# lukecq1231/nats

Hardware: NVIDIA H100
Metric: decoder tokens/sec (dim=1000, src=400, |V|=30k) @1/2/4/8 H100 vs Theano CPU (higher is better)
Workload: dtype f32

## Files before the change

### nats_b200/csrc/api.cu

```cuda
#include <stdarg.h>
#include <stdlib.h>

#include <vector>

#include "model.cuh"

namespace nats {
static thread_local char g_err[1024] = "";
void set_error(const char* fmt, ...) {
    va_list ap;
    va_start(ap, fmt);
    vsnprintf(g_err, sizeof(g_err), fmt, ap);
    va_end(ap);
}
}

namespace nats {
namespace {
struct ProfRec { int cls; double flops, bytes; };
struct ProfState {
    bool on = false;
    std::vector<cudaEvent_t> ev;
    std::vector<ProfRec> recs;
};
// ... 312 lines not shown

int64_t nats_sampler_workspace_bytes(const nats_dims_t* dims, int Tx, int n) {
    if (check_dims(dims) != 0 || Tx < 1 || n < 1) return -1;
    return carve_sampler(*dims, Tx, n, nullptr).bytes;
}

int nats_sampler_init(nats_ctx_t* ctx, void* stream, const nats_dims_t* dims, const float* params, const int64_t* x,
                      const float* x_mask, int Tx, int n, void* ws, int64_t ws_bytes, float* init_state, float* ctx_out,
                      float* pctx_out) {
    NATS_REQUIRE(ctx && ws && params && x && init_state && ctx_out, "null argument");
    NATS_TRY(check_dims(dims));
    NATS_REQUIRE(Tx >= 1 && n >= 1, "shape");
    const SamplerWS w = carve_sampler(*dims, Tx, n, ws);
    NATS_REQUIRE(ws_bytes >= w.bytes, "workspace too small (see nats_sampler_workspace_bytes)");
    cudaStream_t st = reinterpret_cast<cudaStream_t>(stream);
    EncBufs e;
    memset(&e, 0, sizeof(e));
    e.emb_x = w.emb_x;
    e.xproj[0] = w.xproj[0]; e.xproj[1] = w.xproj[1];
    e.cc = ctx_out; e.ctxsum = w.ctxsum; e.xlen = w.xlen; e.xinv = w.xinv; e.ctx_mean = w.ctx_mean;
    e.init_state = init_state; e.part_a = w.part_a;
    e.gemm_scratch = w.gemm_scratch; e.gemm_scratch_floats = w.gemm_scratch_floats;
    e.enc_scratch = w.enc_scratch; e.enc_scratch_floats = w.enc_scratch_floats;
    e.enc_counters = w.enc_counters; e.enc_counter_ints = w.enc_counter_ints;
    NATS_TRY(encoder_forward(ctx, st, *dims, params, x, x_mask, Tx, n, e));
    if (pctx_out) {
        const ParamOff o = param_offsets(*dims);
        const int A = dims->dim_att, C = 2 * dims->dim;
        GemmProblem p = gemm_problem(ctx_out, C, params + o.Wc_att, A, pctx_out, A, Tx * n, A, C);
        p.bias = params + o.b_att;
        NATS_TRY(gemm_auto(ctx, st, p, false, false, w.gemm_scratch, w.gemm_scratch_floats));
    }
    return 0;
}

}

namespace {

int sampler_next(nats_ctx_t* ctx, void* stream, const nats_dims_t* dims, const float* params, const int64_t* y,
                 const float* ctx_in, int64_t ctx_tstride, int64_t ctx_bstride, const float* pctx_in,
                 int64_t pctx_tstride, int64_t pctx_bstride, int rows_per_src, const int32_t* src_len, const float* state,
                 const float* acc_ctx, const float* acc_alpha, int Tx, int n, uint64_t rng_seed, uint64_t rng_step, void* ws,
                 int64_t ws_bytes, float* probs, int64_t* sample, float* state_out, float* alphaT, float* ctxs,
                 float* acc_ctx_out, float* acc_alpha_out) {
    NATS_REQUIRE(ctx && ws && params && y && ctx_in && state && acc_ctx && acc_alpha, "null argument");
    NATS_REQUIRE(probs && state_out && alphaT && ctxs && acc_ctx_out && acc_alpha_out, "null output");
// ... 225 lines not shown
```

### nats_b200/csrc/enc_tc.cu

```cuda
#include <cuda.h>

#include "ops.cuh"
#include "tc_common.cuh"

namespace nats {

namespace {

using namespace tc;

constexpr int kMmaWG = 3;
constexpr int kMmaThreads = kMmaWG * 128;
constexpr int kProdWarp = kMmaWG * 4;
constexpr int kGateWarp0 = kProdWarp + 1;
constexpr int kGateThreads = 256;
constexpr int kThreads = kGateWarp0 * 32 + kGateThreads;
constexpr int kMaxRows = 64 * kMmaWG;
constexpr int kMaxNS = 8;
constexpr int kMaxWords = 12;
constexpr int kMaxDps = 16;
constexpr int kMaxCtasPerDir = 74;
constexpr long long kSpinLimit = 2000000000LL;
constexpr int kCtrStride = 32;

struct EncTc {
    CUtensorMap map_raw[2];
    CUtensorMap map_lo[2];
    const float* Ucat[2];
    const float* mask;
    const float* xproj[2];
    float* cc;
    float* r[2]; float* u[2]; float* c[2]; float* p[2];
    float* ctxsum;
    const float* dcc;
    const float* mean_grad;
    const float* coef;
    float* dG[2]; float* dGx[2];
    float* lo;
    unsigned long long* slab;
    unsigned* bar;
    unsigned long long* dbg;
    int Tx, n, D, Kp;
    int NT, S, dpc, dps, Kc, nkbA, NS, nwg;
};

__device__ __forceinline__ void mbar_wait_b(uint64_t* bar, uint32_t parity) {
    const uint32_t addr = smem_u32(bar);
    const long long t0 = clock64();
    uint32_t ok;
    do {
        asm volatile(
            "{\n\t.reg .pred p;\n\t"
            "mbarrier.try_wait.parity.shared::cta.b64 p, [%1], %2;\n\t"
            "selp.u32 %0, 1, 0, p;\n\t}"
            : "=r"(ok) : "r"(addr), "r"(parity) : "memory");
        if (!ok && clock64() - t0 > kSpinLimit) __trap();
    } while (!ok);
}
__device__ __forceinline__ void flag_arrive(unsigned* ctr) {
    asm volatile("red.release.gpu.global.add.u32 [%0], 1;" ::"l"(ctr) : "memory");
}
// ... 4 lines not shown
__device__ __forceinline__ unsigned long long ld_word(const unsigned long long* p) {
    unsigned long long w;
    asm volatile("ld.relaxed.gpu.global.u64 %0, [%1];" : "=l"(w) : "l"(p) : "memory");
    return w;
}

__device__ __forceinline__ uint32_t a_off(int m, int k, uint32_t kb_bytes) {
    const int kb = k >> 5, kk = k & 31;
    return (uint32_t)kb * kb_bytes + (uint32_t)m * 128u + (uint32_t)(((kk >> 2) ^ (m & 7)) << 4) + (uint32_t)((kk & 3) << 2);
}

template <int BN>
__device__ __forceinline__ void mma_ss(float (&d)[BN / 2], uint64_t da, uint64_t db) {
    if constexpr (BN == 32) wgmma_ss_n32(d, da, db);
    else wgmma_ss_n64(d, da, db);
}
template <int BN>
__device__ __forceinline__ void mma_rs(float (&d)[BN / 2], const uint32_t (&a)[4], uint64_t db) {
    if constexpr (BN == 32) wgmma_rs_n32(d, a, db);
    else wgmma_rs_n64(d, a, db);
}

template <int BN, bool BWD>
__global__ void __launch_bounds__(kThreads, 1) enc_tc_kernel(const __grid_constant__ EncTc a) {
    constexpr uint32_t kStage = 2u * BN * 128u;
    constexpr int EPT = (kMaxDps * BN + kGateThreads - 1) / kGateThreads;
    constexpr int NG = BWD ? 1 : 3;
    constexpr int R = BN / 2;

    extern __shared__ __align__(1024) unsigned char smem[];
    __shared__ __align__(8) uint64_t full[kMaxNS];
    __shared__ __align__(8) uint64_t empty[kMaxNS];

    const int tid = threadIdx.x, warp = __shfl_sync(0xffffffffu, tid >> 5, 0), lane = tid & 31;
    const int D = a.D, n = a.n, Tx = a.Tx, D3 = 3 * a.D, C = 2 * a.D;
    const int S = a.S, NT = a.NT, dpc = a.dpc, dps = a.dps;
    const int dir = blockIdx.x / (NT * S);
    const int rem = blockIdx.x - dir * NT * S;
    const int tile = rem / S, crank = rem - tile * S;
    const int d0 = tile * dpc;
    const int nd = min(dpc, D - d0);
    const int Ktot = BWD ? D3 : D;
    const int kbeg = crank * a.Kc;
    const int kend = min(Ktot, kbeg + a.Kc);
    const int klen = max(0, kend - kbeg);
    const int nkb = (klen + 31) >> 5;
    const int NS = a.NS;
    const uint32_t kb_bytes = (uint32_t)a.nwg * 8192u;

    const uint32_t sA = (smem_u32(smem) + 1023u) & ~1023u;
    const uint32_t sRing = sA + (uint32_t)a.nkbA * kb_bytes;

    {
        const uint32_t words = (uint32_t)a.nkbA * kb_bytes / 4u;
        for (uint32_t i = tid; i < words / 4; i += kThreads)
            asm volatile("st.shared.v4.f32 [%0], {%1,%1,%1,%1};" ::"r"(sA + i * 16u), "f"(0.f) : "memory");
    }
    if (tid == 0) {
        asm volatile("prefetch.tensormap [%0];" ::"l"(&a.map_raw[dir]) : "memory");
        asm volatile("prefetch.tensormap [%0];" ::"l"(&a.map_lo[dir]) : "memory");
        for (int s = 0; s < NS; ++s) { mbar_init(&full[s], 1); mbar_init(&empty[s], kMmaThreads / 32); }
        asm volatile("fence.mbarrier_init.release.cluster;" ::: "memory");
    }
    __syncthreads();
    {
        const float* __restrict__ W = a.Ucat[dir];
        if (!BWD) {
            const int rows = 3 * nd;
            const int total = klen * rows;
            for (int e = tid; e < total; e += kThreads) {
                const int kl = e / rows, mm = e - kl * rows;
                const int g = mm / nd, dl = mm - g * nd;
                const float v = __ldg(W + (long long)(kbeg + kl) * D3 + g * D + d0 + dl);
                asm volatile("st.shared.f32 [%0], %1;" ::"r"(sA + a_off(g * dpc + dl, kl, kb_bytes)), "f"(v) : "memory");
            }
        } else {
            const int total = nd * klen;
            for (int e = tid; e < total; e += kThreads) {
                const int m = e / klen, kl = e - m * klen;
                const float v = __ldg(W + (long long)(d0 + m) * D3 + kbeg + kl);
                asm volatile("st.shared.f32 [%0], %1;" ::"r"(sA + a_off(m, kl, kb_bytes)), "f"(v) : "memory");
            }
        }
    }
    asm volatile("fence.proxy.async.shared::cta;" ::: "memory");
    __syncthreads();

    unsigned* tctr = a.bar + (dir * NT + tile) * kCtrStride;
    const bool stamp = a.dbg != nullptr && blockIdx.x == 0;
#define ENC_STAMP(i) do { a.dbg[i] = gtimer(); a.dbg[32 + (i)] = (unsigned long long)clock64(); } while (0)

    if (warp == kProdWarp) {
        const int kcov = min(Ktot, kbeg + 32 * nkb);
        bool need = false;
        if (lane < NT) {
            const int u0 = lane * dpc, u1 = min(D, u0 + dpc);
            for (int g = 0; g < (BWD ? 3 : 1); ++g) need = need || (g * D + u0 < kcov && g * D + u1 > kbeg);
        }
        const unsigned* pctr = a.bar + (dir * NT + lane) * kCtrStride;
        uint32_t it = 0;
        for (int s = 1; s < Tx; ++s) {
            {
                const unsigned target = (unsigned)(S * (kGateThreads / 32) * s);
                const long long t0 = clock64();
                bool ok;
                do {
                    ok = true;
                    if (need) {
                        unsigned v;
                        asm volatile("ld.acquire.gpu.global.u32 %0, [%1];" : "=r"(v) : "l"(pctr) : "memory");
                        ok = v >= target;
                    }
                    if (!ok && clock64() - t0 > kSpinLimit) __trap();
                } while (!__all_sync(0xffffffffu, ok));
            }
            if (lane == 0) {
                const int brow = BWD ? (dir == 0 ? Tx - s : s - 1) : (dir == 0 ? s - 1 : Tx - s);
                asm volatile("fence.proxy.async;" ::: "memory");
                if (stamp && s == 8) ENC_STAMP(0);
                for (int kb = 0; kb < nkb; ++kb, ++it) {
                    const uint32_t slot = it % (uint32_t)NS;
                    if (it >= (uint32_t)NS) mbar_wait_b(&empty[slot], ((it / (uint32_t)NS) - 1u) & 1u);
                    mbar_expect_tx(&full[slot], kStage);
                    const uint32_t dst = sRing + slot * kStage;
                    tma_load_3d(dst, &a.map_raw[dir], &full[slot], kbeg + 32 * kb, 0, brow);
                    tma_load_3d(dst + BN * 128u, &a.map_lo[dir], &full[slot], kbeg + 32 * kb, 0, (s - 1) & 1);
                }
            }
            __syncwarp();
        }
    } else if (warp < kProdWarp) {
        const int wg = warp >> 2;
        const bool active = wg < a.nwg;
        const int r0 = 64 * wg + 16 * (warp & 3) + (lane >> 2);
        const int q = lane & 3;
        int g_row[2], dl_row[2];
        bool row_ok[2];
        unsigned long long* slab_w[2];
#pragma unroll
        for (int h = 0; h < 2; ++h) {
// ... 43 lines not shown
                    wgmma_commit();
                    wgmma_wait<0>();
                    reg_fence(acc_hh); reg_fence(acc_x);
                }
                __syncwarp();
                if (lane == 0) mbar_arrive(&empty[slot]);
            }
            if (stamp && s == 8 && tid == 0) ENC_STAMP(3);
#pragma unroll
            for (int h = 0; h < 2; ++h) {
                if (!row_ok[h]) continue;
#pragma unroll
                for (int j = 0; j < BN / 8; ++j)
#pragma unroll
                    for (int e = 0; e < 2; ++e) {
                        const int i = 4 * j + 2 * h + e;
                        st_word(slab_w[h] + (long long)(8 * j + 2 * q + e) * dpc, acc_hh[i] + acc_x[i], (uint32_t)s);
                    }
            }
            if (stamp && s == 8 && tid == 0) ENC_STAMP(6);
            asm volatile("bar.arrive 2, %0;" ::"r"(kMmaThreads + kGateThreads) : "memory");
        }
    } else {
        const int gtid = tid - kGateWarp0 * 32;
        const unsigned long long* slab_tile = a.slab + (long long)(dir * NT + tile) * S * NG * BN * dpc;
        const int nw = S * NG;
        const int nds = max(0, min(dps, nd - crank * dps));
        const int dbase = d0 + crank * dps;
        int eb[EPT], ed[EPT];
        bool ev[EPT];
        float carry[EPT], csum[EPT];
#pragma unroll
        for (int i = 0; i < EPT; ++i) {
            const int e = gtid + kGateThreads * i;
            eb[i] = e / dps;
            ed[i] = e - eb[i] * dps;
            ev[i] = eb[i] < n && ed[i] < nds;
            carry[i] = 0.f; csum[i] = 0.f;
        }
        for (int s = 0; s < Tx; ++s) {
            const int pos = BWD ? (dir == 0 ? Tx - 1 - s : s) : (dir == 0 ? s : Tx - 1 - s);
            float x0[EPT], x1[EPT], x2[EPT], mk[EPT];
            float sr_[EPT], su_[EPT], sc_[EPT], sp_[EPT];
#pragma unroll
            for (int i = 0; i < EPT; ++i) {
                x0[i] = x1[i] = x2[i] = 0.f; mk[i] = 1.f;
                sr_[i] = su_[i] = sc_[i] = sp_[i] = 0.f;
                if (ev[i]) {
                    const long long row = (long long)pos * n + eb[i];
                    const int d = dbase + ed[i];
                    if (a.mask) mk[i] = __ldg(a.mask + row);
                    if (!BWD) {
                        const float* xp = a.xproj[dir] + row * D3 + d;
                        x0[i] = __ldg(xp); x1[i] = __ldg(xp + D); x2[i] = __ldg(xp + 2 * D);
                    } else {
                        const long long o = row * D + d;
                        sr_[i] = __ldg(a.r[dir] + o); su_[i] = __ldg(a.u[dir] + o); sc_[i] = __ldg(a.c[dir] + o); sp_[i] = __ldg(a.p[dir] + o);
                        x0[i] = __ldg(a.dcc + row * C + dir * D + d);
                        const int prev = dir == 0 ? pos - 1 : pos + 1;
                        x1[i] = (s < Tx - 1) ? __ldg(a.cc + ((long long)prev * n + eb[i]) * C + dir * D + d) : 0.f;
                        x2[i] = a.mean_grad ? __ldg(a.coef + eb[i]) * __ldg(a.mean_grad + (long long)eb[i] * C + dir * D + d) : 0.f;
                    }
                }
            }
            constexpr bool kDefer = EPT <= 2;
            float o0[kDefer ? EPT : 1], o1[kDefer ? EPT : 1], o2[kDefer ? EPT : 1], o3[kDefer ? EPT : 1];
            auto finish = [&](int i, float s0, float s1, float s2) {
                const long long row = (long long)pos * n + eb[i];
                const int d = dbase + ed[i];
                float q0, q1, q2, q3 = 0.f;
                if (!BWD) {
                    const float r = sigmoidf_(s0 + x0[i]), u = sigmoidf_(s1 + x1[i]);
                    const float cnd = tanhf(s2 * r + x2[i]);
                    const float hn = u * carry[i] + (1.f - u) * cnd;
                    const float h = mk[i] * hn + (1.f - mk[i]) * carry[i];
                    a.cc[row * C + dir * D + d] = h;
                    a.lo[((long long)(dir * 2 + (s & 1)) * n + eb[i]) * a.Kp + d] = resid(h);
                    carry[i] = h;
                    csum[i] += mk[i] * h;
                    q0 = r; q1 = u; q2 = cnd; q3 = s2;
                } else {
                    const float m = mk[i], r = sr_[i], u = su_[i], cnd = sc_[i], pp = sp_[i], hp = x1[i];
                    float dh = x0[i];
                    if (s > 0) { dh += carry[i]; dh += s0; }
                    if (a.mean_grad) dh += m * x2[i];
                    const float dhn = m * dh;
                    const float du = dhn * (hp - cnd);
                    const float dc = dhn * (1.f - u);
                    const float dpc_ = dc * (1.f - cnd * cnd);
                    const float dp = dpc_ * r;
                    const float dr = dpc_ * pp;
                    const float dgr = dr * r * (1.f - r);
                    const float dgu = du * u * (1.f - u);
                    float* g = a.dG[dir] + row * D3 + d;
                    g[0] = dgr; g[D] = dgu; g[2 * D] = dp;
                    float* gl = a.lo + ((long long)(dir * 2 + (s & 1)) * n + eb[i]) * a.Kp + d;
                    gl[0] = resid(dgr); gl[D] = resid(dgu); gl[2 * D] = resid(dp);
                    carry[i] = (1.f - m) * dh + dhn * u;
                    q0 = dgr; q1 = dgu; q2 = dpc_;
                }
// ... 46 lines not shown
                    for (int j = 0; j < 2; ++j) {
                        if (i0 + j < EPT && ev[i0 + j]) {
                            float p0 = 0.f, p1 = 0.f, p2 = 0.f;
#pragma unroll
                            for (int k = 0; k < kMaxWords; k += NG) {
                                if (k < nw) {
                                    p0 += __uint_as_float((uint32_t)w[j][k]);
                                    if (NG == 3) {
                                        p1 += __uint_as_float((uint32_t)w[j][k + NG - 2]);
                                        p2 += __uint_as_float((uint32_t)w[j][k + NG - 1]);
                                    }
                                }
                            }
                            finish(i0 + j, p0, p1, p2);
                        }
                    }
                }
            } else {
#pragma unroll
                for (int i = 0; i < EPT; ++i)
                    if (ev[i]) finish(i, 0.f, 0.f, 0.f);
            }
            if (stamp && s == 8 && gtid == 0) ENC_STAMP(9);
            __syncwarp();
            if (lane == 0) {
                flag_arrive(tctr);
                if (stamp && s == 8 && gtid == 0) ENC_STAMP(5);
            }
            if (kDefer) {
#pragma unroll
                for (int i = 0; i < EPT; ++i) {
                    if (ev[i]) {
                        const long long row = (long long)pos * n + eb[i];
                        const int d = dbase + ed[i];
                        if (!BWD) {
                            if (a.r[dir]) {
                                const long long o = row * D + d;
                                a.r[dir][o] = o0[kDefer ? i : 0]; a.u[dir][o] = o1[kDefer ? i : 0];
                                a.c[dir][o] = o2[kDefer ? i : 0]; a.p[dir][o] = o3[kDefer ? i : 0];
                            }
                        } else {
                            float* gx = a.dGx[dir] + row * D3 + d;
                            gx[0] = o0[kDefer ? i : 0]; gx[D] = o1[kDefer ? i : 0]; gx[2 * D] = o2[kDefer ? i : 0];
                        }
                    }
                }
            }
        }
        if (!BWD && a.ctxsum) {
#pragma unroll
            for (int i = 0; i < EPT; ++i)
                if (ev[i]) a.ctxsum[(long long)eb[i] * C + dir * D + dbase + ed[i]] = csum[i];
        }
    }
}

typedef CUresult (*EncodeTiledFn)(CUtensorMap*, CUtensorMapDataType, cuuint32_t, void*, const cuuint64_t*, const cuuint64_t*,
                                  const cuuint32_t*, const cuuint32_t*, CUtensorMapInterleave, CUtensorMapSwizzle,
                                  CUtensorMapL2promotion, CUtensorMapFloatOOBfill);
EncodeTiledFn g_enc = nullptr;
int g_enable = 1;
size_t g_static_smem = 1024;
int g_resident = -1;

int make_map(const float* ptr, long long inner, long long rows, long long outer, long long row_stride, long long outer_stride,
             int box_rows, CUtensorMap* out) {
    cuuint64_t gdim[3] = {(cuuint64_t)inner, (cuuint64_t)rows, (cuuint64_t)outer};
    cuuint64_t gstr[2] = {(cuuint64_t)row_stride * 4, (cuuint64_t)outer_stride * 4};
    cuuint32_t box[3] = {32, (cuuint32_t)box_rows, 1};
    cuuint32_t estr[3] = {1, 1, 1};
    const CUresult r = g_enc(out, CU_TENSOR_MAP_DATA_TYPE_FLOAT32, 3, const_cast<float*>(ptr), gdim, gstr, box, estr,
                             CU_TENSOR_MAP_INTERLEAVE_NONE, CU_TENSOR_MAP_SWIZZLE_128B, CU_TENSOR_MAP_L2_PROMOTION_L2_128B,
                             CU_TENSOR_MAP_FLOAT_OOB_FILL_NONE);
    if (r != CUDA_SUCCESS) {
        set_error("enc_tc: cuTensorMapEncodeTiled failed (%d): ptr=%p inner=%lld rows=%lld outer=%lld", (int)r, ptr, inner, rows, outer);
        return 1;
    }
    return 0;
}

struct TcPlan {
    bool ok;
    int BN, NT, S, NG, dpc, dps, Kc, nkbA, NS, Ktot, nwg;
    size_t smem;
    long long slab_floats, lo_floats, counter_ints;
};

TcPlan plan(const nats_ctx* ctx, int n, int D, int pass) {
    TcPlan p;
    memset(&p, 0, sizeof(p));
    if (g_enc == nullptr || n < 1 || n > 64 || D < 96 || (D & 3)) return p;
    p.BN = n <= 32 ? 32 : 64;
    const int per_dir = min(ctx->num_sms / 2, kMaxCtasPerDir);
    const size_t lim = (size_t)ctx->max_smem_optin - g_static_smem - 1024;
    const size_t stage = (size_t)2 * p.BN * 128;
    p.NG = pass == 0 ? 3 : 1;
    p.Ktot = pass == 0 ? D : 3 * D;
    TcPlan best = p;
    for (int S = 2; S <= kMaxWords / p.NG; ++S) {
        const int NT0 = per_dir / S;
        if (NT0 < 1) break;
        const int dpc = (D + NT0 - 1) / NT0;
        const int NT = (D + dpc - 1) / dpc;
        const int rows = p.NG * dpc;
        if (rows > kMaxRows || NT > 32) continue;
        const int dps = (dpc + S - 1) / S;
        if (dps > kMaxDps) continue;
        const int Kc = (((p.Ktot + S - 1) / S + 31) / 32) * 32;
        if (p.Ktot - Kc * (S - 1) < 8) continue;
        const int nwg = (rows + 63) / 64;
        const size_t fixed = (size_t)(Kc / 32) * nwg * 8192;
        if (fixed + 2 * stage > lim) continue;
        if (best.ok && Kc / 32 >= best.nkbA) continue;
        p.S = S; p.NT = NT; p.dpc = dpc; p.dps = dps; p.Kc = Kc; p.nkbA = Kc / 32; p.nwg = nwg;
        p.NS = (int)((lim - fixed) / stage);
        if (p.NS > kMaxNS) p.NS = kMaxNS;
        if (p.NS > p.nkbA) p.NS = max(2, p.nkbA);
        p.smem = fixed + (size_t)p.NS * stage + 1024;
        const long long Kp = (p.Ktot + 3) / 4 * 4;
        p.lo_floats = (4LL * n * Kp + 3) / 4 * 4;
        p.slab_floats = 2LL * (2LL * p.NT * p.S * p.NG * p.BN * p.dpc);
        p.counter_ints = 2LL * p.NT * kCtrStride;
        p.ok = true;
        best = p;
    }
    return best;
}

template <int BN, bool BWD>
int launch(cudaStream_t st, const TcPlan& pl, const EncTc& a) {
    enc_tc_kernel<BN, BWD><<<dim3(2 * pl.NT * pl.S), dim3(kThreads), pl.smem, st>>>(a);
    NATS_LAUNCH_OK();
    return 0;
}

}

void enc_tc_enable(int on) { g_enable = on; }

int enc_tc_setup(const nats_ctx* ctx) {
    void* fn = nullptr;
    cudaDriverEntryPointQueryResult q;
    NATS_CUDA_OK(cudaGetDriverEntryPoint("cuTensorMapEncodeTiled", &fn, cudaEnableDefault, &q));
    if (fn == nullptr || q != cudaDriverEntryPointSuccess) return 0;
    cudaFuncAttributes fa;
    size_t st = 0;
    NATS_CUDA_OK(cudaFuncGetAttributes(&fa, enc_tc_kernel<32, false>)); st = st > fa.sharedSizeBytes ? st : fa.sharedSizeBytes;
    NATS_CUDA_OK(cudaFuncGetAttributes(&fa, enc_tc_kernel<64, false>)); st = st > fa.sharedSizeBytes ? st : fa.sharedSizeBytes;
    NATS_CUDA_OK(cudaFuncGetAttributes(&fa, enc_tc_kernel<32, true>)); st = st > fa.sharedSizeBytes ? st : fa.sharedSizeBytes;
    NATS_CUDA_OK(cudaFuncGetAttributes(&fa, enc_tc_kernel<64, true>)); st = st > fa.sharedSizeBytes ? st : fa.sharedSizeBytes;
    g_static_smem = st;
    const int dyn = ctx->max_smem_optin - (int)g_static_smem;
    NATS_CUDA_OK(cudaFuncSetAttribute(enc_tc_kernel<32, false>, cudaFuncAttributeMaxDynamicSharedMemorySize, dyn));
    NATS_CUDA_OK(cudaFuncSetAttribute(enc_tc_kernel<64, false>, cudaFuncAttributeMaxDynamicSharedMemorySize, dyn));
    NATS_CUDA_OK(cudaFuncSetAttribute(enc_tc_kernel<32, true>, cudaFuncAttributeMaxDynamicSharedMemorySize, dyn));
    NATS_CUDA_OK(cudaFuncSetAttribute(enc_tc_kernel<64, true>, cudaFuncAttributeMaxDynamicSharedMemorySize, dyn));
    int r = 0;
    NATS_CUDA_OK(cudaOccupancyMaxActiveBlocksPerMultiprocessor(&r, enc_tc_kernel<32, false>, kThreads, dyn));
    g_resident = r;
    g_enc = reinterpret_cast<EncodeTiledFn>(fn);
    return 0;
}

bool enc_tc_eligible(const nats_ctx* ctx, int n, int D, int pass) {
    if (!(g_enable == 1 || (g_enable == 2 && pass == 0) || (g_enable == 3 && pass == 1))) return false;
    if (g_resident < 1) return false;
    const TcPlan p = plan(ctx, n, D, pass);
    return p.ok && 2 * p.NT * p.S <= ctx->num_sms;
}

long long enc_tc_scratch_floats(int n, int D) {
    const long long BN = n <= 32 ? 32 : 64;
    return 4LL * n * (3LL * D + 4) + 2LL * (2LL * kMaxCtasPerDir * kMaxRows * BN) + 64;
}
long long enc_tc_counter_ints() { return 2LL * 32 * kCtrStride + 64; }

int enc_tc_fwd(const nats_ctx* ctx, cudaStream_t st, const EncTcFwdArgs& g) {
    const TcPlan pl = plan(ctx, g.n, g.D, 0);
    NATS_REQUIRE(pl.ok && 2 * pl.NT * pl.S <= ctx->num_sms, "tensor-core persistent encoder not applicable");
    NATS_REQUIRE((reinterpret_cast<uintptr_t>(g.cc) & 15) == 0 && (reinterpret_cast<uintptr_t>(g.scratch) & 15) == 0, "alignment");
    NATS_REQUIRE(g.scratch_floats >= pl.lo_floats + pl.slab_floats && g.bar_ints >= pl.counter_ints, "scratch size");
    EncTc a;
    memset(&a, 0, sizeof(a));
    const int D = g.D, n = g.n, Kp = (D + 3) / 4 * 4;
    for (int d = 0; d < 2; ++d) {
        a.Ucat[d] = g.Ucat[d]; a.xproj[d] = g.xproj[d];
        a.r[d] = g.r[d]; a.u[d] = g.u[d]; a.c[d] = g.c[d]; a.p[d] = g.p[d];
        NATS_TRY(make_map(g.cc + (long long)d * D, D, n, g.Tx, 2LL * D, 2LL * D * n, pl.BN, &a.map_raw[d]));
        NATS_TRY(make_map(g.scratch + (long long)d * 2 * n * Kp, D, n, 2, Kp, (long long)n * Kp, pl.BN, &a.map_lo[d]));
    }
    a.mask = g.mask; a.cc = g.cc; a.lo = g.scratch; a.slab = reinterpret_cast<unsigned long long*>(g.scratch + pl.lo_floats); a.ctxsum = g.ctxsum; a.bar = g.bar; a.dbg = g.dbg;
    a.Tx = g.Tx; a.n = n; a.D = D; a.Kp = Kp;
    a.NT = pl.NT; a.S = pl.S; a.dpc = pl.dpc; a.dps = pl.dps; a.Kc = pl.Kc; a.nkbA = pl.nkbA; a.NS = pl.NS; a.nwg = pl.nwg;
    NATS_CUDA_OK(memset_async(st, g.bar, 0, (size_t)pl.counter_ints * sizeof(unsigned)));
    NATS_CUDA_OK(memset_async(st, g.scratch + pl.lo_floats, 0xff, (size_t)pl.slab_floats * sizeof(float)));
    ProfScope ps(st, K_ENC_PERSIST_FWD, 2.0 * 2 * g.Tx * (double)n * 3.0 * D * D, 4.0 * 2 * 3.0 * D * D);
    return pl.BN == 32 ? launch<32, false>(st, pl, a) : launch<64, false>(st, pl, a);
}

int enc_tc_bwd(const nats_ctx* ctx, cudaStream_t st, const EncTcBwdArgs& g) {
    const TcPlan pl = plan(ctx, g.n, g.D, 1);
    NATS_REQUIRE(pl.ok && 2 * pl.NT * pl.S <= ctx->num_sms, "tensor-core persistent encoder (backward) not applicable");
    NATS_REQUIRE((reinterpret_cast<uintptr_t>(g.dG[0]) & 15) == 0 && (reinterpret_cast<uintptr_t>(g.dG[1]) & 15) == 0 &&
                     (reinterpret_cast<uintptr_t>(g.scratch) & 15) == 0, "alignment");
    NATS_REQUIRE(g.scratch_floats >= pl.lo_floats + pl.slab_floats && g.bar_ints >= pl.counter_ints, "scratch size");
    EncTc a;
    memset(&a, 0, sizeof(a));
    const int D = g.D, n = g.n, K = 3 * D, Kp = (K + 3) / 4 * 4;
    for (int d = 0; d < 2; ++d) {
        a.Ucat[d] = g.Ucat[d];
        a.r[d] = const_cast<float*>(g.r[d]); a.u[d] = const_cast<float*>(g.u[d]);
        a.c[d] = const_cast<float*>(g.c[d]); a.p[d] = const_cast<float*>(g.p[d]);
        a.dG[d] = g.dG[d]; a.dGx[d] = g.dGx[d];
        NATS_TRY(make_map(g.dG[d], K, n, g.Tx, K, (long long)K * n, pl.BN, &a.map_raw[d]));
        NATS_TRY(make_map(g.scratch + (long long)d * 2 * n * Kp, K, n, 2, Kp, (long long)n * Kp, pl.BN, &a.map_lo[d]));
    }
    a.mask = g.mask; a.cc = const_cast<float*>(g.cc); a.dcc = g.dcc; a.mean_grad = g.mean_grad; a.coef = g.coef;
    a.lo = g.scratch; a.slab = reinterpret_cast<unsigned long long*>(g.scratch + pl.lo_floats); a.bar = g.bar; a.dbg = g.dbg;
    a.Tx = g.Tx; a.n = n; a.D = D; a.Kp = Kp;
    a.NT = pl.NT; a.S = pl.S; a.dpc = pl.dpc; a.dps = pl.dps; a.Kc = pl.Kc; a.nkbA = pl.nkbA; a.NS = pl.NS; a.nwg = pl.nwg;
    NATS_CUDA_OK(memset_async(st, g.bar, 0, (size_t)pl.counter_ints * sizeof(unsigned)));
    NATS_CUDA_OK(memset_async(st, g.scratch + pl.lo_floats, 0xff, (size_t)pl.slab_floats * sizeof(float)));
    ProfScope ps(st, K_ENC_PERSIST_BWD, 2.0 * 2 * g.Tx * (double)n * 3.0 * D * D, 4.0 * 2 * 3.0 * D * D);
    return pl.BN == 32 ? launch<32, true>(st, pl, a) : launch<64, true>(st, pl, a);
}

}
```

### nats_b200/csrc/model.cuh

```cuda
#pragma once
#include "common.cuh"
#include "gemm.cuh"
#include "ops.cuh"
#include "workspace.cuh"

namespace nats {

struct EncBufs {
    float* emb_x;
    float* xproj[2];
    float* r[2]; float* u[2]; float* c[2]; float* p[2];
    float* cc;
    float* ctxsum; float* xlen; float* xinv; float* ctx_mean; float* init_state;
    float* part_a;
    float* gemm_scratch; long long gemm_scratch_floats;
    float* enc_scratch; long long enc_scratch_floats;
    unsigned* enc_counters; long long enc_counter_ints;
};
int encoder_forward(const nats_ctx* ctx, cudaStream_t st, const nats_dims_t& d, const float* params,
                    const int64_t* x, const float* x_mask, int Tx, int n, const EncBufs& e);

struct DecStep {
    int n, Tx;
    const float* h_prev;
    const float* xproj;
    const float* ymask;
    const float* xmask;
    int rows_per_src;
    const int32_t* src_len;
    const float* pctx; long long pctx_ts, pctx_bs;
    const float* cc; long long cc_ts, cc_bs;
    const float* acc_alpha_in; const float* acc_ctx_in;
    float* h1; float* r1; float* u1; float* c1; float* p1;
    float* ps_save; float* escore;
    float* alpha_out; float* acc_alpha_out; float* craw_out; float* ctx_out; float* acc_ctx_out;
    float* r2; float* u2; float* c2; float* p2; float* h2;
    float* part_a; float* part_b; float* part_c; float* part_d;
};
int decoder_step_forward(const nats_ctx* ctx, cudaStream_t st, const nats_dims_t& d, const float* params,
                         const DecStep& s);
// ... 20 lines not shown
```

### nats_b200/csrc/model_fwd.cu

```cuda
#include "model.cuh"

namespace nats {

int encoder_forward(const nats_ctx* ctx, cudaStream_t st, const nats_dims_t& d, const float* params,
                    const int64_t* x, const float* x_mask, int Tx, int n, const EncBufs& e) {
    const ParamOff o = param_offsets(d);
    const int W = d.dim_word, D = d.dim, V = d.n_words, C = 2 * D, D3 = 3 * D;
    const long long XB = (long long)Tx * n;
    NATS_TRY(gather_rows(st, params + o.Wemb, x, (int)XB, W, V, 0, e.emb_x));
    {
        GemmProblem pr[2];
        for (int dir = 0; dir < 2; ++dir) {
            pr[dir] = gemm_problem(e.emb_x, W, params + o.enc[dir].Wcat, D3, e.xproj[dir], D3, (int)XB, D3, W);
            pr[dir].bias = params + o.enc[dir].bcat;
        }
        NATS_TRY(gemm_launch(st, pr, 2, false, false, GEMM_CFG_AUTO));
    }
    NATS_CUDA_OK(memset_async(st, e.ctxsum, 0, (size_t)n * C * sizeof(float)));
    const int S = gemm_pick_split(ctx, n, D3, D, 2);
    const int cfg = gemm_step_cfg(n);
    const long long strideP = 2LL * n * D3;
    if (enc_tc_eligible(ctx, n, D, 0) && e.enc_scratch != nullptr) {
        EncTcFwdArgs pa;
        memset(&pa, 0, sizeof(pa));
        for (int dir = 0; dir < 2; ++dir) {
            pa.Ucat[dir] = params + o.enc[dir].Ucat; pa.xproj[dir] = e.xproj[dir];
            pa.r[dir] = e.r[dir]; pa.u[dir] = e.u[dir]; pa.c[dir] = e.c[dir]; pa.p[dir] = e.p[dir];
        }
        pa.mask = x_mask; pa.cc = e.cc; pa.ctxsum = e.ctxsum;
        pa.bar = e.enc_counters; pa.bar_ints = e.enc_counter_ints;
        pa.scratch = e.enc_scratch; pa.scratch_floats = e.enc_scratch_floats;
        pa.Tx = Tx; pa.n = n; pa.D = D;
        NATS_TRY(enc_tc_fwd(ctx, st, pa));
    } else {
        for (int s = 0; s < Tx; ++s) {
            const int pf = s, pb = Tx - 1 - s;
            if (s > 0) {
                GemmProblem q[2];
                q[0] = gemm_problem(e.cc + (long long)(pf - 1) * n * C, C, params + o.enc[0].Ucat, D3, e.part_a, D3, n, D3, D);
                q[1] = gemm_problem(e.cc + (long long)(pb + 1) * n * C + D, C, params + o.enc[1].Ucat, D3,
                                    e.part_a + (long long)n * D3, D3, n, D3, D);
                gemm_set_split(q[0], S, strideP);
                gemm_set_split(q[1], S, strideP);
                NATS_TRY(gemm_launch(st, q, 2, false, false, cfg));
            }
            GateFwd g[2];
            memset(g, 0, sizeof(g));
            for (int dir = 0; dir < 2; ++dir) {
                const int pos = dir == 0 ? pf : pb;
                const int prev = dir == 0 ? pf - 1 : pb + 1;
                g[dir].part = e.part_a + (long long)dir * n * D3;
                g[dir].nsplit = s > 0 ? S : 0;
                g[dir].part_stride = strideP;
// ... 81 lines not shown
        g.bias = params + o.b1cat;
        g.h_prev = s.h1; g.ld_hprev = D;
        g.mask = s.ymask;
        g.h_out = s.h2; g.ld_hout = D;
        g.r = s.r2; g.u = s.u2; g.c = s.c2; g.p = s.p2;
        NATS_TRY(gru_gates_fwd(st, &g, 1, n, D, 1));
    }
    return 0;
}

int train_encoder_fwd(const nats_ctx* ctx, cudaStream_t st, const nats_dims_t& d, const float* params,
                      const int64_t* x, const float* x_mask, int Tx, int B, const TrainWS& w) {
    EncBufs e;
    memset(&e, 0, sizeof(e));
    e.emb_x = w.emb_x;
    for (int i = 0; i < 2; ++i) {
        e.xproj[i] = w.xproj[i];
        e.r[i] = w.enc_r[i]; e.u[i] = w.enc_u[i]; e.c[i] = w.enc_c[i]; e.p[i] = w.enc_p[i];
    }
    e.cc = w.cc; e.ctxsum = w.ctxsum; e.xlen = w.xlen; e.xinv = w.xinv; e.ctx_mean = w.ctx_mean;
    e.init_state = w.init_state; e.part_a = w.part_a;
    e.gemm_scratch = w.gemm_scratch; e.gemm_scratch_floats = w.gemm_scratch_floats;
    e.enc_scratch = w.enc_scratch; e.enc_scratch_floats = w.enc_scratch_floats;
    e.enc_counters = w.enc_counters; e.enc_counter_ints = w.enc_counter_ints;
    return encoder_forward(ctx, st, d, params, x, x_mask, Tx, B, e);
}

int train_decoder_fwd(const nats_ctx* ctx, cudaStream_t st, const nats_dims_t& d, const float* params,
                      const int64_t* y, const float* x_mask, const float* y_mask, int Tx, int Ty, int B,
                      const TrainWS& w) {
    const ParamOff o = param_offsets(d);
    const int W = d.dim_word, D = d.dim, A = d.dim_att, V = d.n_words, C = 2 * D, D3 = 3 * D;
    const long long XB = (long long)Tx * B, YB = (long long)Ty * B;
    NATS_TRY(gather_rows(st, params + o.Wemb, y, (int)YB, W, V, B, w.embs));
    {
        GemmProblem p = gemm_problem(w.embs, W, params + o.dec.Wcat, D3, w.xproj_y, D3, (int)YB, D3, W);
        p.bias = params + o.dec.bcat;
        NATS_TRY(gemm_auto(ctx, st, p, false, false, w.gemm_scratch, w.gemm_scratch_floats));
    }
    {
        GemmProblem p = gemm_problem(w.cc, C, params + o.Wc_att, A, w.pctx, A, (int)XB, A, C);
        p.bias = params + o.b_att;
        NATS_TRY(gemm_auto(ctx, st, p, false, false, w.gemm_scratch, w.gemm_scratch_floats));
    }
    NATS_CUDA_OK(memset_async(st, w.d_accalpha, 0, (size_t)B * Tx * sizeof(float)));
    NATS_CUDA_OK(memset_async(st, w.d_accctx, 0, (size_t)B * C * sizeof(float)));
    for (int t = 0; t < Ty; ++t) {
// ... 49 lines not shown
```

### nats_b200/csrc/ops.cuh

```cuda
#pragma once
#include "common.cuh"

namespace nats {

int gather_rows(cudaStream_t st, const float* Wemb, const int64_t* ids, int n_rows, int W, int V, int shift,
                float* out);
int scatter_add_rows(cudaStream_t st, float* dWemb, const int64_t* ids, int n_rows, int W, int V, int shift,
                     const float* src);

struct GateFwd {
    const float* part;
    int nsplit;
    long long part_stride;
    const float* xproj;
    const float* part2;
    int nsplit2;
    long long part2_stride;
    const float* bias;
    const float* h_prev;
    int ld_hprev;
    const float* mask;
    float* h_out;
    int ld_hout;
    float* r; float* u; float* c; float* p;
// ... 2 lines not shown
};
int gru_gates_fwd(cudaStream_t st, const GateFwd* groups, int ngroups, int B, int D, int mode);

struct GateBwd {
    const float* dh_a; int ld_a;
    const float* dh_b; int ld_b;
    const float* part;  int nsplit;  long long part_stride;  int part_ld;
    const float* part2; int nsplit2; long long part2_stride; int part2_ld;
    const float* mean_grad; int ld_mean;
    const float* coef;
    const float* r; const float* u; const float* c; const float* p;
    const float* h_prev; int ld_hprev;
    const float* mask;
    float* dG;
    float* dGx;
    float* dh_elem;
};
int gru_gates_bwd(cudaStream_t st, const GateBwd* groups, int ngroups, int B, int D);

struct EncTcFwdArgs {
    const float* Ucat[2]; const float* xproj[2]; const float* mask; float* cc;
    float* r[2]; float* u[2]; float* c[2]; float* p[2];
    float* ctxsum;
    unsigned* bar; long long bar_ints;
    float* scratch; long long scratch_floats;
    unsigned long long* dbg;
    int Tx, n, D;
};
struct EncTcBwdArgs {
    const float* Ucat[2]; const float* dcc; const float* mean_grad; const float* coef; const float* mask; const float* cc;
    const float* r[2]; const float* u[2]; const float* c[2]; const float* p[2];
    float* dG[2]; float* dGx[2];
    unsigned* bar; long long bar_ints; float* scratch; long long scratch_floats;
    unsigned long long* dbg;
    int Tx, n, D;
};
bool enc_tc_eligible(const nats_ctx* ctx, int n, int D, int pass);
void enc_tc_enable(int on);
int enc_tc_setup(const nats_ctx* ctx);
long long enc_tc_scratch_floats(int n, int D);
long long enc_tc_counter_ints();
int enc_tc_fwd(const nats_ctx* ctx, cudaStream_t st, const EncTcFwdArgs& a);
int enc_tc_bwd(const nats_ctx* ctx, cudaStream_t st, const EncTcBwdArgs& a);
void tma_gemm_set_ts(int on);
int tma_gemm_get_ts();
void gates_trace(int on);
void attention_set_cc_keep(int mode);

int tanh_inplace(cudaStream_t st, float* x, long long n);
struct NarrowProj {
    const float* x[3]; long long ldx[3];
    const float* W[3]; long long ldw[3];
    const float* bias[3];
    int K[3];
    int n, N;
    float* out; long long ldo;
// ... 99 lines not shown
```

### nats_b200/csrc/workspace.cuh

```cuda
#pragma once
#include "common.cuh"
#include "gemm.cuh"
#include "ops.cuh"

namespace nats {

struct GruOff { int64_t Wcat, bcat, Ucat; };
struct ParamOff {
    int64_t Wemb;
    GruOff enc[2];
    int64_t ff_state_W, ff_state_b;
    GruOff dec;
    int64_t U1cat, W1cat, b1cat;
    int64_t W_att, Wc_att, b_att, U_att, c_att, W_con, U_con, D_wei;
    int64_t lstm_W, lstm_b, prev_W, prev_b, ctxr_W, ctxr_b, logit_W, logit_b;
    int64_t total;
};

inline ParamOff param_offsets(const nats_dims_t& d) {
    const int64_t V = d.n_words, W = d.dim_word, D = d.dim, A = d.dim_att, C = 2 * D;
    ParamOff o;
    int64_t off = 0;
    auto take = [&](int64_t n) { int64_t r = off; off += round_up64(n, 32); return r; };
    o.Wemb = take(V * W);
// ... 167 lines not shown
struct SamplerWS {
    float* emb_x;
    float* xproj[2];
    float* ctxsum;
    float* ctx_mean;
    float* xlen; float* xinv;
    float* part_a;
    float* part_b;
    float* part_c;
    float* part_d;
    float* emb_y;
    float* xproj_y;
    float* pctx;
    float* escore;
    float* h1;
    float* ps;
    float* craw;
    float* L;
    float* logits;
    float* gemm_scratch;
    int64_t gemm_scratch_floats;
    float* enc_scratch;
    int64_t enc_scratch_floats;
    unsigned* enc_counters;
    int64_t enc_counter_ints;
    int64_t bytes;
};

inline SamplerWS carve_sampler(const nats_dims_t& d, int Tx, int n, void* base) {
    const int64_t W = d.dim_word, D = d.dim, A = d.dim_att, V = d.n_words, C = 2 * D;
    const int64_t XB = (int64_t)Tx * n;
    SamplerWS w;
    memset(&w, 0, sizeof(w));
    Carver c{reinterpret_cast<char*>(base), 0};
    w.emb_x = c.f(XB * W);
    for (int i = 0; i < 2; ++i) w.xproj[i] = c.f(XB * 3 * D);
    w.ctxsum = c.f(n * C); w.ctx_mean = c.f(n * C); w.xlen = c.f(n); w.xinv = c.f(n);
    w.part_a = c.f((int64_t)kStepMaxSplit * 2 * n * 3 * D);
    w.part_b = c.f((int64_t)kStepMaxSplit * n * 3 * D);
    w.part_c = c.f((int64_t)kStepMaxSplit * n * 3 * D);
    w.part_d = c.f((int64_t)kStepMaxSplit * n * (A > D ? A : D));
    w.emb_y = c.f(n * W); w.xproj_y = c.f(n * 3 * D); w.pctx = c.f(XB * A); w.escore = c.f((int64_t)n * Tx);
    w.h1 = c.f(n * D); w.ps = c.f(n * A); w.craw = c.f(n * C); w.L = c.f(n * W); w.logits = c.f(n * V);
    w.gemm_scratch_floats = 4LL << 20;
    w.gemm_scratch = c.f(w.gemm_scratch_floats);
    w.enc_scratch_floats = enc_tc_scratch_floats(n, (int)D);
    w.enc_scratch = c.f(w.enc_scratch_floats);
    w.enc_counter_ints = enc_tc_counter_ints();
    w.enc_counters = c.take<unsigned>(w.enc_counter_ints);
    w.bytes = round_up64(c.off, 256);
    return w;
}

}
```

Before: 32830.

## Replace TMA producer and counters with gate-warp stamped word exchange in forward encoder

```diff
diff --git a/nats_b200/csrc/api.cu b/nats_b200/csrc/api.cu
--- a/nats_b200/csrc/api.cu
+++ b/nats_b200/csrc/api.cu
@@ -358,7 +358,6 @@
     e.init_state = init_state; e.part_a = w.part_a;
     e.gemm_scratch = w.gemm_scratch; e.gemm_scratch_floats = w.gemm_scratch_floats;
     e.enc_scratch = w.enc_scratch; e.enc_scratch_floats = w.enc_scratch_floats;
-    e.enc_counters = w.enc_counters; e.enc_counter_ints = w.enc_counter_ints;
     NATS_TRY(encoder_forward(ctx, st, *dims, params, x, x_mask, Tx, n, e));
     if (pctx_out) {
         const ParamOff o = param_offsets(*dims);
diff --git a/nats_b200/csrc/enc_tc.cu b/nats_b200/csrc/enc_tc.cu
--- a/nats_b200/csrc/enc_tc.cu
+++ b/nats_b200/csrc/enc_tc.cu
@@ -12,9 +12,11 @@
 constexpr int kMmaWG = 3;
 constexpr int kMmaThreads = kMmaWG * 128;
 constexpr int kProdWarp = kMmaWG * 4;
-constexpr int kGateWarp0 = kProdWarp + 1;
 constexpr int kGateThreads = 256;
-constexpr int kThreads = kGateWarp0 * 32 + kGateThreads;
+template <bool BWD>
+constexpr int kGateWarp0 = kProdWarp + (BWD ? 1 : 0);
+template <bool BWD>
+constexpr int kThreads = kGateWarp0<BWD> * 32 + kGateThreads;
 constexpr int kMaxRows = 64 * kMmaWG;
 constexpr int kMaxNS = 8;
 constexpr int kMaxWords = 12;
@@ -37,6 +39,7 @@
     const float* coef;
     float* dG[2]; float* dGx[2];
     float* lo;
+    unsigned long long* xw;
     unsigned long long* slab;
     unsigned* bar;
     unsigned long long* dbg;
@@ -87,11 +90,12 @@
 }
 
 template <int BN, bool BWD>
-__global__ void __launch_bounds__(kThreads, 1) enc_tc_kernel(const __grid_constant__ EncTc a) {
+__global__ void __launch_bounds__(kThreads<BWD>, 1) enc_tc_kernel(const __grid_constant__ EncTc a) {
     constexpr uint32_t kStage = 2u * BN * 128u;
     constexpr int EPT = (kMaxDps * BN + kGateThreads - 1) / kGateThreads;
     constexpr int NG = BWD ? 1 : 3;
     constexpr int R = BN / 2;
+    constexpr int kThr = kThreads<BWD>;
 
     extern __shared__ __align__(1024) unsigned char smem[];
     __shared__ __align__(8) uint64_t full[kMaxNS];
@@ -118,13 +122,15 @@
 
     {
         const uint32_t words = (uint32_t)a.nkbA * kb_bytes / 4u;
-        for (uint32_t i = tid; i < words / 4; i += kThreads)
+        for (uint32_t i = tid; i < words / 4; i += kThr)
             asm volatile("st.shared.v4.f32 [%0], {%1,%1,%1,%1};" ::"r"(sA + i * 16u), "f"(0.f) : "memory");
     }
     if (tid == 0) {
-        asm volatile("prefetch.tensormap [%0];" ::"l"(&a.map_raw[dir]) : "memory");
-        asm volatile("prefetch.tensormap [%0];" ::"l"(&a.map_lo[dir]) : "memory");
-        for (int s = 0; s < NS; ++s) { mbar_init(&full[s], 1); mbar_init(&empty[s], kMmaThreads / 32); }
+        if (BWD) {
+            asm volatile("prefetch.tensormap [%0];" ::"l"(&a.map_raw[dir]) : "memory");
+            asm volatile("prefetch.tensormap [%0];" ::"l"(&a.map_lo[dir]) : "memory");
+        }
+        for (int s = 0; s < NS; ++s) { mbar_init(&full[s], BWD ? 1 : kGateThreads / 32); mbar_init(&empty[s], kMmaThreads / 32); }
         asm volatile("fence.mbarrier_init.release.cluster;" ::: "memory");
     }
     __syncthreads();
@@ -133,7 +139,7 @@
         if (!BWD) {
             const int rows = 3 * nd;
             const int total = klen * rows;
-            for (int e = tid; e < total; e += kThreads) {
+            for (int e = tid; e < total; e += kThr) {
                 const int kl = e / rows, mm = e - kl * rows;
                 const int g = mm / nd, dl = mm - g * nd;
                 const float v = __ldg(W + (long long)(kbeg + kl) * D3 + g * D + d0 + dl);
@@ -141,7 +147,7 @@
             }
         } else {
             const int total = nd * klen;
-            for (int e = tid; e < total; e += kThreads) {
+            for (int e = tid; e < total; e += kThr) {
                 const int m = e / klen, kl = e - m * klen;
                 const float v = __ldg(W + (long long)(d0 + m) * D3 + kbeg + kl);
                 asm volatile("st.shared.f32 [%0], %1;" ::"r"(sA + a_off(m, kl, kb_bytes)), "f"(v) : "memory");
@@ -151,11 +157,11 @@
     asm volatile("fence.proxy.async.shared::cta;" ::: "memory");
     __syncthreads();
 
-    unsigned* tctr = a.bar + (dir * NT + tile) * kCtrStride;
+    unsigned* tctr = BWD ? a.bar + (dir * NT + tile) * kCtrStride : nullptr;
     const bool stamp = a.dbg != nullptr && blockIdx.x == 0;
 #define ENC_STAMP(i) do { a.dbg[i] = gtimer(); a.dbg[32 + (i)] = (unsigned long long)clock64(); } while (0)
 
-    if (warp == kProdWarp) {
+    if (BWD && warp == kProdWarp) {
         const int kcov = min(Ktot, kbeg + 32 * nkb);
         bool need = false;
         if (lane < NT) {
@@ -180,7 +186,7 @@
                 } while (!__all_sync(0xffffffffu, ok));
             }
             if (lane == 0) {
-                const int brow = BWD ? (dir == 0 ? Tx - s : s - 1) : (dir == 0 ? s - 1 : Tx - s);
+                const int brow = dir == 0 ? Tx - s : s - 1;
                 asm volatile("fence.proxy.async;" ::: "memory");
                 if (stamp && s == 8) ENC_STAMP(0);
                 for (int kb = 0; kb < nkb; ++kb, ++it) {
@@ -270,7 +276,8 @@
             asm volatile("bar.arrive 2, %0;" ::"r"(kMmaThreads + kGateThreads) : "memory");
         }
     } else {
-        const int gtid = tid - kGateWarp0 * 32;
+        const int gtid = tid - kGateWarp0<BWD> * 32;
+        const int gw = warp - kGateWarp0<BWD>;
         const unsigned long long* slab_tile = a.slab + (long long)(dir * NT + tile) * S * NG * BN * dpc;
         const int nw = S * NG;
         const int nds = max(0, min(dps, nd - crank * dps));
@@ -286,8 +293,10 @@
             ev[i] = eb[i] < n && ed[i] < nds;
             carry[i] = 0.f; csum[i] = 0.f;
         }
+        uint32_t it = 0;
         for (int s = 0; s < Tx; ++s) {
             const int pos = BWD ? (dir == 0 ? Tx - 1 - s : s) : (dir == 0 ? s : Tx - 1 - s);
+            unsigned long long* xw_s = BWD ? nullptr : a.xw + (long long)(dir * 2 + (s & 1)) * n * a.Kp;
             float x0[EPT], x1[EPT], x2[EPT], mk[EPT];
             float sr_[EPT], su_[EPT], sc_[EPT], sp_[EPT];
 #pragma unroll
@@ -322,8 +331,8 @@
                     const float cnd = tanhf(s2 * r + x2[i]);
                     const float hn = u * carry[i] + (1.f - u) * cnd;
                     const float h = mk[i] * hn + (1.f - mk[i]) * carry[i];
-                    a.cc[row * C + dir * D + d] = h;
-                    a.lo[((long long)(dir * 2 + (s & 1)) * n + eb[i]) * a.Kp + d] = resid(h);
+                    st_word(xw_s + (long long)eb[i] * a.Kp + d, h, (uint32_t)s);
+                    if (!kDefer) a.cc[row * C + dir * D + d] = h;
                     carry[i] = h;
                     csum[i] += mk[i] * h;
                     q0 = r; q1 = u; q2 = cnd; q3 = s2;
@@ -416,10 +425,12 @@
                     if (ev[i]) finish(i, 0.f, 0.f, 0.f);
             }
             if (stamp && s == 8 && gtid == 0) ENC_STAMP(9);
-            __syncwarp();
-            if (lane == 0) {
-                flag_arrive(tctr);
-                if (stamp && s == 8 && gtid == 0) ENC_STAMP(5);
+            if (BWD) {
+                __syncwarp();
+                if (lane == 0) {
+                    flag_arrive(tctr);
+                    if (stamp && s == 8 && gtid == 0) ENC_STAMP(5);
+                }
             }
             if (kDefer) {
 #pragma unroll
@@ -428,6 +439,7 @@
                         const long long row = (long long)pos * n + eb[i];
                         const int d = dbase + ed[i];
                         if (!BWD) {
+                            a.cc[row * C + dir * D + d] = carry[i];
                             if (a.r[dir]) {
                                 const long long o = row * D + d;
                                 a.r[dir][o] = o0[kDefer ? i : 0]; a.u[dir][o] = o1[kDefer ? i : 0];
@@ -438,6 +450,46 @@
                             gx[0] = o0[kDefer ? i : 0]; gx[D] = o1[kDefer ? i : 0]; gx[2 * D] = o2[kDefer ? i : 0];
                         }
                     }
+                }
+            }
+            if (!BWD && s + 1 < Tx) {
+                constexpr int RPW = BN / 8;
+                const unsigned long long* src = xw_s + kbeg + lane;
+                const unsigned long long ready = (unsigned long long)s << 32;
+                auto valid = [&](int kb, int j) { return kb < nkb && kbeg + 32 * kb + lane < Ktot && gw + 8 * j < n; };
+                auto addr = [&](int kb, int j) { return src + (long long)(gw + 8 * j) * a.Kp + 32 * kb; };
+                unsigned long long w[RPW];
+#pragma unroll
+                for (int j = 0; j < RPW; ++j) w[j] = valid(0, j) ? ld_word(addr(0, j)) : ready;
+                for (int kb = 0; kb < nkb; ++kb, ++it) {
+                    const long long t0 = clock64();
+                    for (;;) {
+                        bool stale = false;
+#pragma unroll
+                        for (int j = 0; j < RPW; ++j)
+                            if ((uint32_t)(w[j] >> 32) != (uint32_t)s) { w[j] = ld_word(addr(kb, j)); stale = true; }
+                        if (!stale) break;
+                        if (clock64() - t0 > kSpinLimit) __trap();
+                    }
+                    if (stamp && s + 1 == 8 && kb == 0 && gtid == 0) ENC_STAMP(0);
+                    float v[RPW];
+#pragma unroll
+                    for (int j = 0; j < RPW; ++j) {
+                        v[j] = __uint_as_float((uint32_t)w[j]);
+                        w[j] = valid(kb + 1, j) ? ld_word(addr(kb + 1, j)) : ready;
+                    }
+                    const uint32_t slot = it % (uint32_t)NS;
+                    if (it >= (uint32_t)NS) mbar_wait_b(&empty[slot], ((it / (uint32_t)NS) - 1u) & 1u);
+                    const uint32_t dst = sRing + slot * kStage + (uint32_t)gw * 128u + ((((uint32_t)lane >> 2) ^ (uint32_t)gw) << 4) +
+                                         ((uint32_t)lane & 3u) * 4u;
+#pragma unroll
+                    for (int j = 0; j < RPW; ++j) {
+                        asm volatile("st.shared.f32 [%0], %1;" ::"r"(dst + (uint32_t)j * 1024u), "f"(v[j]) : "memory");
+                        asm volatile("st.shared.f32 [%0], %1;" ::"r"(dst + (uint32_t)j * 1024u + BN * 128u), "f"(resid(v[j])) : "memory");
+                    }
+                    asm volatile("fence.proxy.async.shared::cta;" ::: "memory");
+                    __syncwarp();
+                    if (lane == 0) mbar_arrive(&full[slot]);
                 }
             }
         }
@@ -477,7 +529,7 @@
     bool ok;
     int BN, NT, S, NG, dpc, dps, Kc, nkbA, NS, Ktot, nwg;
     size_t smem;
-    long long slab_floats, lo_floats, counter_ints;
+    long long slab_floats, xfer_floats, counter_ints;
 };
 
 TcPlan plan(const nats_ctx* ctx, int n, int D, int pass) {
@@ -512,9 +564,9 @@
         if (p.NS > p.nkbA) p.NS = max(2, p.nkbA);
         p.smem = fixed + (size_t)p.NS * stage + 1024;
         const long long Kp = (p.Ktot + 3) / 4 * 4;
-        p.lo_floats = (4LL * n * Kp + 3) / 4 * 4;
+        p.xfer_floats = pass == 0 ? 2LL * (4LL * n * Kp) : (4LL * n * Kp + 3) / 4 * 4;
         p.slab_floats = 2LL * (2LL * p.NT * p.S * p.NG * p.BN * p.dpc);
-        p.counter_ints = 2LL * p.NT * kCtrStride;
+        p.counter_ints = pass == 0 ? 0 : 2LL * p.NT * kCtrStride;
         p.ok = true;
         best = p;
     }
@@ -523,7 +575,7 @@
 
 template <int BN, bool BWD>
 int launch(cudaStream_t st, const TcPlan& pl, const EncTc& a) {
-    enc_tc_kernel<BN, BWD><<<dim3(2 * pl.NT * pl.S), dim3(kThreads), pl.smem, st>>>(a);
+    enc_tc_kernel<BN, BWD><<<dim3(2 * pl.NT * pl.S), dim3(kThreads<BWD>), pl.smem, st>>>(a);
     NATS_LAUNCH_OK();
     return 0;
 }
@@ -549,9 +601,10 @@
     NATS_CUDA_OK(cudaFuncSetAttribute(enc_tc_kernel<64, false>, cudaFuncAttributeMaxDynamicSharedMemorySize, dyn));
     NATS_CUDA_OK(cudaFuncSetAttribute(enc_tc_kernel<32, true>, cudaFuncAttributeMaxDynamicSharedMemorySize, dyn));
     NATS_CUDA_OK(cudaFuncSetAttribute(enc_tc_kernel<64, true>, cudaFuncAttributeMaxDynamicSharedMemorySize, dyn));
-    int r = 0;
-    NATS_CUDA_OK(cudaOccupancyMaxActiveBlocksPerMultiprocessor(&r, enc_tc_kernel<32, false>, kThreads, dyn));
-    g_resident = r;
+    int rf = 0, rb = 0;
+    NATS_CUDA_OK(cudaOccupancyMaxActiveBlocksPerMultiprocessor(&rf, enc_tc_kernel<64, false>, kThreads<false>, dyn));
+    NATS_CUDA_OK(cudaOccupancyMaxActiveBlocksPerMultiprocessor(&rb, enc_tc_kernel<64, true>, kThreads<true>, dyn));
+    g_resident = rf < rb ? rf : rb;
     g_enc = reinterpret_cast<EncodeTiledFn>(fn);
     return 0;
 }
@@ -572,22 +625,20 @@
 int enc_tc_fwd(const nats_ctx* ctx, cudaStream_t st, const EncTcFwdArgs& g) {
     const TcPlan pl = plan(ctx, g.n, g.D, 0);
     NATS_REQUIRE(pl.ok && 2 * pl.NT * pl.S <= ctx->num_sms, "tensor-core persistent encoder not applicable");
-    NATS_REQUIRE((reinterpret_cast<uintptr_t>(g.cc) & 15) == 0 && (reinterpret_cast<uintptr_t>(g.scratch) & 15) == 0, "alignment");
-    NATS_REQUIRE(g.scratch_floats >= pl.lo_floats + pl.slab_floats && g.bar_ints >= pl.counter_ints, "scratch size");
+    NATS_REQUIRE((reinterpret_cast<uintptr_t>(g.scratch) & 15) == 0, "alignment");
+    NATS_REQUIRE(g.scratch_floats >= pl.xfer_floats + pl.slab_floats, "scratch size");
     EncTc a;
     memset(&a, 0, sizeof(a));
-    const int D = g.D, n = g.n, Kp = (D + 3) / 4 * 4;
+    const int D = g.D, n = g.n;
     for (int d = 0; d < 2; ++d) {
         a.Ucat[d] = g.Ucat[d]; a.xproj[d] = g.xproj[d];
         a.r[d] = g.r[d]; a.u[d] = g.u[d]; a.c[d] = g.c[d]; a.p[d] = g.p[d];
-        NATS_TRY(make_map(g.cc + (long long)d * D, D, n, g.Tx, 2LL * D, 2LL * D * n, pl.BN, &a.map_raw[d]));
-        NATS_TRY(make_map(g.scratch + (long long)d * 2 * n * Kp, D, n, 2, Kp, (long long)n * Kp, pl.BN, &a.map_lo[d]));
-    }
-    a.mask = g.mask; a.cc = g.cc; a.lo = g.scratch; a.slab = reinterpret_cast<unsigned long long*>(g.scratch + pl.lo_floats); a.ctxsum = g.ctxsum; a.bar = g.bar; a.dbg = g.dbg;
-    a.Tx = g.Tx; a.n = n; a.D = D; a.Kp = Kp;
+    }
+    a.mask = g.mask; a.cc = g.cc; a.ctxsum = g.ctxsum; a.dbg = g.dbg;
+    a.xw = reinterpret_cast<unsigned long long*>(g.scratch); a.slab = reinterpret_cast<unsigned long long*>(g.scratch + pl.xfer_floats);
+    a.Tx = g.Tx; a.n = n; a.D = D; a.Kp = (D + 3) / 4 * 4;
     a.NT = pl.NT; a.S = pl.S; a.dpc = pl.dpc; a.dps = pl.dps; a.Kc = pl.Kc; a.nkbA = pl.nkbA; a.NS = pl.NS; a.nwg = pl.nwg;
-    NATS_CUDA_OK(memset_async(st, g.bar, 0, (size_t)pl.counter_ints * sizeof(unsigned)));
-    NATS_CUDA_OK(memset_async(st, g.scratch + pl.lo_floats, 0xff, (size_t)pl.slab_floats * sizeof(float)));
+    NATS_CUDA_OK(memset_async(st, g.scratch, 0xff, (size_t)(pl.xfer_floats + pl.slab_floats) * sizeof(float)));
     ProfScope ps(st, K_ENC_PERSIST_FWD, 2.0 * 2 * g.Tx * (double)n * 3.0 * D * D, 4.0 * 2 * 3.0 * D * D);
     return pl.BN == 32 ? launch<32, false>(st, pl, a) : launch<64, false>(st, pl, a);
 }
@@ -597,7 +648,7 @@
     NATS_REQUIRE(pl.ok && 2 * pl.NT * pl.S <= ctx->num_sms, "tensor-core persistent encoder (backward) not applicable");
     NATS_REQUIRE((reinterpret_cast<uintptr_t>(g.dG[0]) & 15) == 0 && (reinterpret_cast<uintptr_t>(g.dG[1]) & 15) == 0 &&
                      (reinterpret_cast<uintptr_t>(g.scratch) & 15) == 0, "alignment");
-    NATS_REQUIRE(g.scratch_floats >= pl.lo_floats + pl.slab_floats && g.bar_ints >= pl.counter_ints, "scratch size");
+    NATS_REQUIRE(g.scratch_floats >= pl.xfer_floats + pl.slab_floats && g.bar_ints >= pl.counter_ints, "scratch size");
     EncTc a;
     memset(&a, 0, sizeof(a));
     const int D = g.D, n = g.n, K = 3 * D, Kp = (K + 3) / 4 * 4;
@@ -610,11 +661,11 @@
         NATS_TRY(make_map(g.scratch + (long long)d * 2 * n * Kp, K, n, 2, Kp, (long long)n * Kp, pl.BN, &a.map_lo[d]));
     }
     a.mask = g.mask; a.cc = const_cast<float*>(g.cc); a.dcc = g.dcc; a.mean_grad = g.mean_grad; a.coef = g.coef;
-    a.lo = g.scratch; a.slab = reinterpret_cast<unsigned long long*>(g.scratch + pl.lo_floats); a.bar = g.bar; a.dbg = g.dbg;
+    a.lo = g.scratch; a.slab = reinterpret_cast<unsigned long long*>(g.scratch + pl.xfer_floats); a.bar = g.bar; a.dbg = g.dbg;
     a.Tx = g.Tx; a.n = n; a.D = D; a.Kp = Kp;
     a.NT = pl.NT; a.S = pl.S; a.dpc = pl.dpc; a.dps = pl.dps; a.Kc = pl.Kc; a.nkbA = pl.nkbA; a.NS = pl.NS; a.nwg = pl.nwg;
     NATS_CUDA_OK(memset_async(st, g.bar, 0, (size_t)pl.counter_ints * sizeof(unsigned)));
-    NATS_CUDA_OK(memset_async(st, g.scratch + pl.lo_floats, 0xff, (size_t)pl.slab_floats * sizeof(float)));
+    NATS_CUDA_OK(memset_async(st, g.scratch + pl.xfer_floats, 0xff, (size_t)pl.slab_floats * sizeof(float)));
     ProfScope ps(st, K_ENC_PERSIST_BWD, 2.0 * 2 * g.Tx * (double)n * 3.0 * D * D, 4.0 * 2 * 3.0 * D * D);
     return pl.BN == 32 ? launch<32, true>(st, pl, a) : launch<64, true>(st, pl, a);
 }
diff --git a/nats_b200/csrc/model.cuh b/nats_b200/csrc/model.cuh
--- a/nats_b200/csrc/model.cuh
+++ b/nats_b200/csrc/model.cuh
@@ -15,7 +15,6 @@
     float* part_a;
     float* gemm_scratch; long long gemm_scratch_floats;
     float* enc_scratch; long long enc_scratch_floats;
-    unsigned* enc_counters; long long enc_counter_ints;
 };
 int encoder_forward(const nats_ctx* ctx, cudaStream_t st, const nats_dims_t& d, const float* params,
                     const int64_t* x, const float* x_mask, int Tx, int n, const EncBufs& e);
diff --git a/nats_b200/csrc/model_fwd.cu b/nats_b200/csrc/model_fwd.cu
--- a/nats_b200/csrc/model_fwd.cu
+++ b/nats_b200/csrc/model_fwd.cu
@@ -28,7 +28,6 @@
             pa.r[dir] = e.r[dir]; pa.u[dir] = e.u[dir]; pa.c[dir] = e.c[dir]; pa.p[dir] = e.p[dir];
         }
         pa.mask = x_mask; pa.cc = e.cc; pa.ctxsum = e.ctxsum;
-        pa.bar = e.enc_counters; pa.bar_ints = e.enc_counter_ints;
         pa.scratch = e.enc_scratch; pa.scratch_floats = e.enc_scratch_floats;
         pa.Tx = Tx; pa.n = n; pa.D = D;
         NATS_TRY(enc_tc_fwd(ctx, st, pa));
@@ -156,7 +155,6 @@
     e.init_state = w.init_state; e.part_a = w.part_a;
     e.gemm_scratch = w.gemm_scratch; e.gemm_scratch_floats = w.gemm_scratch_floats;
     e.enc_scratch = w.enc_scratch; e.enc_scratch_floats = w.enc_scratch_floats;
-    e.enc_counters = w.enc_counters; e.enc_counter_ints = w.enc_counter_ints;
     return encoder_forward(ctx, st, d, params, x, x_mask, Tx, B, e);
 }
 
diff --git a/nats_b200/csrc/ops.cuh b/nats_b200/csrc/ops.cuh
--- a/nats_b200/csrc/ops.cuh
+++ b/nats_b200/csrc/ops.cuh
@@ -48,7 +48,6 @@
     const float* Ucat[2]; const float* xproj[2]; const float* mask; float* cc;
     float* r[2]; float* u[2]; float* c[2]; float* p[2];
     float* ctxsum;
-    unsigned* bar; long long bar_ints;
     float* scratch; long long scratch_floats;
     unsigned long long* dbg;
     int Tx, n, D;
@@ -57,7 +56,8 @@
     const float* Ucat[2]; const float* dcc; const float* mean_grad; const float* coef; const float* mask; const float* cc;
     const float* r[2]; const float* u[2]; const float* c[2]; const float* p[2];
     float* dG[2]; float* dGx[2];
-    unsigned* bar; long long bar_ints; float* scratch; long long scratch_floats;
+    unsigned* bar; long long bar_ints;
+    float* scratch; long long scratch_floats;
     unsigned long long* dbg;
     int Tx, n, D;
 };
diff --git a/nats_b200/csrc/workspace.cuh b/nats_b200/csrc/workspace.cuh
--- a/nats_b200/csrc/workspace.cuh
+++ b/nats_b200/csrc/workspace.cuh
@@ -213,8 +213,6 @@
     int64_t gemm_scratch_floats;
     float* enc_scratch;
     int64_t enc_scratch_floats;
-    unsigned* enc_counters;
-    int64_t enc_counter_ints;
     int64_t bytes;
 };
 
@@ -237,8 +235,6 @@
     w.gemm_scratch = c.f(w.gemm_scratch_floats);
     w.enc_scratch_floats = enc_tc_scratch_floats(n, (int)D);
     w.enc_scratch = c.f(w.enc_scratch_floats);
-    w.enc_counter_ints = enc_tc_counter_ints();
-    w.enc_counters = c.take<unsigned>(w.enc_counter_ints);
     w.bytes = round_up64(c.off, 256);
     return w;
 }
```

After: 32720, median of 6. Within noise of the previous version (-0.3%).
